# pennucci/PulsePortraiture

Hardware: AMD Instinct MI355X
Metric: subint_fits_per_sec (higher is better)
Workload: dtype f64

## Files before the change

pulseportraiture_amd/csrc/pp_common.h:

```cpp
#pragma once
#include <hip/hip_runtime.h>
#include <stdint.h>
#include <type_traits>

namespace pp {

#define PP_DCONST 4149.377593360996
#define PP_TWO_PI 6.283185307179586476925286766559
#define PP_LN10 2.302585092994045684017991454684

typedef double2 cplx;

__device__ __forceinline__ cplx cmul(cplx a, cplx b) {
    return make_double2(fma(a.x, b.x, -a.y * b.y), fma(a.x, b.y, a.y * b.x));
}
__device__ __forceinline__ cplx cmulc(cplx a, cplx b) {
    return make_double2(fma(a.x, b.x, a.y * b.y), fma(a.y, b.x, -a.x * b.y));
}
__device__ __forceinline__ cplx cadd(cplx a, cplx b) { return make_double2(a.x + b.x, a.y + b.y); }
__device__ __forceinline__ cplx csub(cplx a, cplx b) { return make_double2(a.x - b.x, a.y - b.y); }
__device__ __forceinline__ cplx cmul_mi(cplx a) { return make_double2(a.y, -a.x); }
__device__ __forceinline__ double cnorm(cplx a) { return fma(a.x, a.x, a.y * a.y); }

template <typename T>
__device__ __forceinline__ const T* as_global(const T* p) {
    typedef const T __attribute__((address_space(1)))* gp_t;
    return (const T*)(gp_t)(uintptr_t)p;
}

template <typename T>
__device__ __forceinline__ T load_uniform(const T* p) {
    typedef const T __attribute__((address_space(4)))* cp_t;
    return *(cp_t)(uintptr_t)p;
}

__device__ __forceinline__ double rn_pin(double r) { asm volatile("" : "+v"(r)); return r; }
__device__ __forceinline__ double mul_rn(double a, double b) { return rn_pin(a * b); }
__device__ __forceinline__ double add_rn(double a, double b) { return rn_pin(a + b); }
__device__ __forceinline__ double sub_rn(double a, double b) { return rn_pin(a - b); }

__device__ __forceinline__ double recip_ge1(double x) {
    double y = __builtin_amdgcn_rcp(x);
    y = fma(fma(-x, y, 1.0), y, y);
    y = fma(fma(-x, y, 1.0), y, y);
    return (x < 1e300) ? y : 0.0;
}

template <bool SC>
__device__ __forceinline__ double kconst(double v) {
    if (SC) asm volatile("" : "+s"(v));
    return v;
}
template <bool SC = false>
__device__ __forceinline__ void sincos_turns(double t, double* sn, double* cs) {
    const double q = rint(4.0 * t);
    const double y = fma(-0.25, q, t);
    const double u = y * y;
    double ps = kconst<SC>(0x1.aaec32af93359p-4);
    ps = fma(ps, u, kconst<SC>(-0x1.6fadb9f155744p-1));
    ps = fma(ps, u, kconst<SC>(0x1.e8f434d018d63p+1));
    ps = fma(ps, u, kconst<SC>(-0x1.e3074fde8871fp+3));
    ps = fma(ps, u, kconst<SC>(0x1.50783487ee782p+5));
    ps = fma(ps, u, kconst<SC>(-0x1.32d2cce62bd86p+6));
    ps = fma(ps, u, kconst<SC>(0x1.466bc6775aae2p+6));
    ps = fma(ps, u, kconst<SC>(-0x1.4abbce625be53p+5));
    ps = fma(ps, u, kconst<SC>(0x1.921fb54442d18p+2));
    const double s0 = ps * y;
    double pc = kconst<SC>(0x1.20c62c2f2d7f5p-2);
    pc = fma(pc, u, kconst<SC>(-0x1.b6e24f44b128fp+0));
    pc = fma(pc, u, kconst<SC>(0x1.f9d38a3763cc3p+2));
    pc = fma(pc, u, kconst<SC>(-0x1.a6d1f2a204a8cp+4));
    pc = fma(pc, u, kconst<SC>(0x1.e1f506891babbp+5));
    pc = fma(pc, u, kconst<SC>(-0x1.55d3c7e3cbffap+6));
    pc = fma(pc, u, kconst<SC>(0x1.03c1f081b5ac4p+6));
    pc = fma(pc, u, kconst<SC>(-0x1.3bd3cc9be45dep+4));
    const double c0 = fma(pc, u, 1.0);
    const int qi = (int)q;
    const bool odd = qi & 1;
    const double so = odd ? c0 : s0, co = odd ? s0 : c0;
    *sn = (qi & 2) ? -so : so;
    *cs = ((qi + 1) & 2) ? -co : co;
}

template <bool SC = false>
__device__ __forceinline__ cplx unit_phasor(double k, double phi) {
    double pfrac = phi - rint(phi);
    double prod = k * pfrac;
    double err = fma(k, pfrac, -prod);
    double r = (prod - rint(prod)) + err;
    double s, c;
    sincos_turns<SC>(r, &s, &c);
    return make_double2(c, s);
}

template <int W>
__device__ __forceinline__ double group_sum(double v) {
#pragma unroll
    for (int o = W / 2; o > 0; o >>= 1) v += __shfl_xor(v, o, 64);
    return v;
}
template <int W>
__device__ __forceinline__ double group_max(double v) {
#pragma unroll
    for (int o = W / 2; o > 0; o >>= 1) v = fmax(v, __shfl_xor(v, o, 64));
    return v;
}

__device__ __forceinline__ int wave_reduce16_index(int lane) { return (lane >> 2) & 15; }
template <int NS>
__device__ __forceinline__ double wave_reduce16(const double (&s)[NS], int lane) {
    double t8[8], t4[4], t2[2];
    const bool b5 = lane & 32, b4 = lane & 16, b3 = lane & 8, b2 = lane & 4;
#pragma unroll
    for (int j = 0; j < 8; ++j) {
        const double hi = (j + 8 < NS) ? s[j + 8] : 0.0;
        const double keep = b5 ? hi : s[j], send = b5 ? s[j] : hi;
        t8[j] = keep + __shfl_xor(send, 32, 64);
    }
#pragma unroll
    for (int j = 0; j < 4; ++j) {
        const double keep = b4 ? t8[j + 4] : t8[j], send = b4 ? t8[j] : t8[j + 4];
        t4[j] = keep + __shfl_xor(send, 16, 64);
    }
#pragma unroll
    for (int j = 0; j < 2; ++j) {
        const double keep = b3 ? t4[j + 2] : t4[j], send = b3 ? t4[j] : t4[j + 2];
        t2[j] = keep + __shfl_xor(send, 8, 64);
    }
    const double keep = b2 ? t2[1] : t2[0], send = b2 ? t2[0] : t2[1];
    double v = keep + __shfl_xor(send, 4, 64);
    v += __shfl_xor(v, 2, 64);
    v += __shfl_xor(v, 1, 64);
    return v;
}

template <int NS>
__device__ __forceinline__ double wave_reduce_lds(const double (&s)[NS], int lane, double* buf) {
    static_assert(NS <= 16, "one value per lane quad");
    const int wpos = (lane >> 4) * 17 + (lane & 15);
#pragma unroll
    for (int q = 0; q < NS; ++q) buf[q * 68 + wpos] = s[q];
    const int q = min(lane >> 2, NS - 1), part = lane & 3;
    const double* src = buf + q * 68 + part * 17;
    double v = 0.0;
#pragma unroll
    for (int t = 0; t < 16; ++t) v += src[t];
    v += __shfl_xor(v, 1, 64);
    v += __shfl_xor(v, 2, 64);
    return v;
}
#define PP_WRED_DOUBLES(NS) ((NS) * 68)

template <int NV>
__device__ inline void block_sum(double (&v)[NV], double* scratch) {
    const int lane = threadIdx.x & 63, wid = threadIdx.x >> 6, nw = blockDim.x >> 6;
#pragma unroll
    for (int i = 0; i < NV; ++i) v[i] = group_sum<64>(v[i]);
    __syncthreads();
    if (lane == 0) {
#pragma unroll
        for (int i = 0; i < NV; ++i) scratch[wid * NV + i] = v[i];
    }
    __syncthreads();
#pragma unroll
    for (int i = 0; i < NV; ++i) {
        double s = 0.0;
        for (int w = 0; w < nw; ++w) s += scratch[w * NV + i];
        v[i] = s;
    }
}

template <int NV, int C0>
__device__ __forceinline__ void wave_totals_to(const double (&v)[NV], int lane, double* dst) {
    constexpr int n = (NV - C0) < 16 ? (NV - C0) : 16;
    double part[n];
#pragma unroll
    for (int j = 0; j < n; ++j) part[j] = v[C0 + j];
    const double tot = wave_reduce16<n>(part, lane);
    if ((lane & 3) == 0 && (lane >> 2) < n) dst[C0 + (lane >> 2)] = tot;
    if constexpr (C0 + 16 < NV) wave_totals_to<NV, C0 + 16>(v, lane, dst);
}
#define PP_BSUM_DOUBLES(NW, NVMAX) (2 * (NW) * ((NVMAX) + 1))
template <int NV, int NVMAX>
__device__ __forceinline__ void block_sum_t(double (&v)[NV], double* scratch, int& flip, double* mx = nullptr) {
    static_assert(NV <= NVMAX, "scratch sized for NVMAX values");
    const int lane = threadIdx.x & 63, wid = threadIdx.x >> 6, nw = blockDim.x >> 6;
    double* buf = scratch + flip * nw * (NVMAX + 1);
    flip ^= 1;
    wave_totals_to<NV, 0>(v, lane, buf + wid * (NV + 1));
    if (mx) {
        const double m = group_max<64>(*mx);
        if (lane == 0) buf[wid * (NV + 1) + NV] = m;
    }
    __syncthreads();
#pragma unroll
    for (int i = 0; i < NV; ++i) {
        double s = 0.0;
        for (int w = 0; w < nw; ++w) s += buf[w * (NV + 1) + i];
        v[i] = s;
    }
    if (mx) {
        double m = buf[NV];
        for (int w = 1; w < nw; ++w) m = fmax(m, buf[w * (NV + 1) + NV]);
        *mx = m;
    }
}

struct SubState {
    double x[5];
    double xe[5];
    double f;
    double g[5];
    double H[25];
    double f0, g0[5], H0[25];
    double radius;
    double pred_red;
    int hits_boundary;
    int iter, nfev, status, done, cur;
    int npass;
    double xl[5], fl, gl[5], Hl[25];
    int fresh;
    int recentred;
    int nmodel;
    int model;
    double xprev[5];
    double geo[4];
};

#define PP_NACC 21
constexpr int PP_CHUNK_CHANNELS = 256;
#define PP_NCS 9
#define PP_TJ 10
#define PP_TSTRIDE (PP_TJ + 2)
#define PP_TAY_PAIR_STRIDE 2
__device__ __forceinline__ size_t tay_idx(size_t row, int q) { return row * PP_TSTRIDE + (size_t)q; }

}
```

pulseportraiture_amd/csrc/pp_xspec1024q.h:

```cpp
#pragma once
#include "pp_fftq.h"


namespace pp {

constexpr unsigned PP_TICKET_WINDOW_NUM = 3u, PP_TICKET_WINDOW_DEN = 4u;
__device__ __forceinline__ int ticket_moment(const long long nrows) {
    const unsigned share = (unsigned)(nrows / (long long)gridDim.x) + 1u;
    return 1 + (int)(((blockIdx.x * 2654435761u) >> 8) % (share * PP_TICKET_WINDOW_NUM / PP_TICKET_WINDOW_DEN + 1u));
}

template <int M, typename Tin>
__device__ __forceinline__ const Tin* next_row_of(const XspecArgs& a, const unsigned more_nx, const int i_nx, const int n_nx,
                                                  const size_t rc) {
    const size_t rn = more_nx ? (size_t)sub_of(a.act, i_nx) * a.nchan_full + (a.coff + n_nx * a.cstep) : rc;
    return reinterpret_cast<const Tin*>(a.data) + rn * (2 * M);
}

constexpr int FFTQ_FREE_ELEM0 = 3 * 272 + 16, FFTQ_FREE_PITCH = 17;

template <int M, bool TAIL, bool ONE = true>
__device__ __forceinline__ void store_row_results(const XspecArgs& a, const size_t rc, const int tid, double tv) {
    constexpr int H = M + 1, kc = (int)(0.75 * H);
  if constexpr (ONE) {
    const int q = wave_reduce16_index(tid);
    const double th = 0.5 * tv;
    double val = (q <= PP_TJ && ((q & 3) == 1 || (q & 3) == 2)) ? -th : th;
    double* dst = a.tay + tay_idx(rc, q < PP_TSTRIDE ? q : 0);
    if (q >= PP_TSTRIDE) { val = tv; dst = a.sdraw + rc; }
    if (TAIL) {
        const double nz = sqrt(tv / (2.0 * M) / (double)(H - kc));
        if (q > PP_TSTRIDE) { val = nz; dst = a.noise + rc; }
    }
    typedef double __attribute__((address_space(1)))* gdp_t;
    *(gdp_t)(uintptr_t)dst = val;
  } else {
    if ((tid & 3) == 0) {
        const int q = wave_reduce16_index(tid);
        if (q < PP_TSTRIDE) {
            tv *= 0.5;
            a.tay[tay_idx(rc, q)] = (q <= PP_TJ && ((q & 3) == 1 || (q & 3) == 2)) ? -tv : tv;
        }
    }
    if (tid == 4 * PP_TSTRIDE) a.sdraw[rc] = tv;
    if (TAIL && tid == 4 * (PP_TSTRIDE + 1)) a.noise[rc] = sqrt(tv / (2.0 * M) / (double)(H - kc));
  }
}

__device__ __forceinline__ void first_row_landed() { __builtin_amdgcn_s_waitcnt(0x0F70); }

constexpr int Q_PREFETCH_F64 = 1, Q_PREFETCH_F32 = 0;
template <typename Tin, bool TAIL>
__global__ __launch_bounds__(64, 2) void k_xspec_q1024(XspecArgs a) {
    constexpr int M = 1024, T = 64, R1 = 16, PER1 = 1;
    constexpr int NSL = 7;
    typedef typename RawOf<Tin>::type Raw;
    constexpr int NRED = PP_TSTRIDE + (TAIL ? 2 : 1);
    static_assert(NRED <= 16, "wave_reduce_lds takes 16 values");
    constexpr int WRED = PP_WRED_DOUBLES(NRED) / 2;
    constexpr int LDSN = WRED > FFTQ_LDS_ELEMS ? WRED : FFTQ_LDS_ELEMS;
    static_assert(2 * LDSN >= PP_TAIL_LDS_DOUBLES, "tail_work's layout of this kernel's LDS");
    constexpr bool F64 = sizeof(Tin) == 8;
    constexpr int NML = (F64 && TAIL) ? 2 : 0;
    constexpr bool TWL = F64 && !TAIL, TWR = F64 && TAIL;
    constexpr bool ROWTOP = !TAIL;
    constexpr int NTW = TWL ? 2 : 0;
    __shared__ cplx lds[LDSN + 64 * (NML + NTW)];
    static_assert(sizeof(lds) <= 19456, "eight workgroups per CU");
    static_assert(FFTQ_FREE_ELEM0 + 15 * FFTQ_FREE_PITCH < FFTQ_LDS_ELEMS && FFTQ_FREE_ELEM0 >= 64 * (TAIL ? 12 : 7) &&
                  2 * FFTQ_FREE_ELEM0 >= PP_WRED_DOUBLES(NRED), "t2's elements are outside everything a row writes");
    cplx* const ldsm = lds + LDSN + threadIdx.x;
    int tid = threadIdx.x;
    const long long nrows = (long long)a.nsub * a.nchan;
    Raw cur[PER1][R1];
    cplx t1 = a.twB[2 * tid], t2 = a.twB[32 * (tid & 15)];
    const int lam0 = fftq_lambda(tid);
    cplx wb0 = a.twB[lam0 ? lam0 : 64];
    const cplx wbT = a.twB[64];
    cplx* const ldt2 = lds + FFTQ_FREE_ELEM0;
    cplx* const ldtw = lds + LDSN + 64 * NML;
    auto put_lane_consts = [&](const cplx p1, const cplx p2, const cplx pb) {
        if (!TWL) return;
        ldt2[FFTQ_FREE_PITCH * (tid & 15)] = p2;
        ldtw[tid] = p1;
        ldtw[64 + tid] = pb;
        lds_sync<T>();
    };
    put_lane_consts(t1, t2, wb0);
    int tail_after = 0x7fffffff;
    if (a.tail) tail_after = ticket_moment(nrows);
    RowWalk<true> rw;
    rw.start(nrows, a.mwords, a.ticket, a.ticket_base);
    long long row = rw.row;
    int n = 0, i = 0;
    if (rw.more) {
        n = __builtin_amdgcn_readfirstlane((int)(row / a.nsub));
        i = __builtin_amdgcn_readfirstlane((int)(row % a.nsub));
        const size_t rc = (size_t)sub_of(a.act, i) * a.nchan_full + (a.coff + n * a.cstep);
        stage_load_global<M, T, R1>(cur, reinterpret_cast<const Tin*>(a.data) + rc * (2 * M), tid);
    }
    cplx mv2[NSL];
    const cplx* mheld = nullptr;
    const cplx* mrow = nullptr;
    int n_held = -1, ktn = 0;
    int i_nx = i, n_nx = n;
    if (ROWTOP) first_row_landed();
#pragma unroll 1
    for (int phase = 0; phase < 2; ++phase) {
    if (phase == 1) {
        if (!a.tail) break;
        tail_work(a.tail, reinterpret_cast<double*>(lds), 2 * (LDSN + 64 * NML), tid, 1);
        tail_after = 0x7fffffff;
        if (TWL) {
            const int lamr = fftq_lambda(tid);
            put_lane_consts(as_global(a.twB)[2 * tid], as_global(a.twB)[32 * (tid & 15)], as_global(a.twB)[lamr ? lamr : 64]);
        }
    }
    for (; rw.more && tail_after != 0; rw.advance(), row = rw.row, i = i_nx, n = n_nx, --tail_after) {
        rw.draw(a.ticket);
        rw.peek(nrows, a.ticket_base, a.mwords);
        asm volatile("" : "+v"(tid));
        const int lam = fftq_lambda(tid);
        const bool l0 = (lam == 0);
        const int kb = l0 ? 64 : lam;
        if (TWR) {
            t1 = as_global(a.twB)[2 * tid];
            t2 = as_global(a.twB)[32 * (tid & 15)];
            wb0 = as_global(a.twB)[kb];
        } else if (!TWL) {
            asm volatile("" : "+v"(t1.x), "+v"(t1.y), "+v"(t2.x), "+v"(t2.y), "+v"(wb0.x), "+v"(wb0.y));
        }
        const int ia = sub_of(a.act, i), ne = a.coff + n * a.cstep;
        const size_t rc = (size_t)ia * a.nchan_full + ne;
        if (channel_lookup(a, ia, n, ne, M, n_held, mrow, ktn) && mrow != mheld) {
#pragma unroll
            for (int j = 0; j < NSL; ++j) {
                const cplx mval = mrow[kb + 64 * j - 1];
                if (j < NSL - NML) mv2[j] = mval; else ldsm[64 * (j - (NSL - NML))] = mval;
            }
            mheld = mrow;
        }
        const double phin = ROWTOP ? load_uniform(a.ph0 + rc) : a.ph0[rc];
        double sd = 0.0;
        cplx v[R1];
#pragma unroll
        for (int k = 0; k < R1; ++k) v[k] = to_cplx(cur[0][k]);
        constexpr bool HALVES = F64;
        const Tin* nxrow = nullptr;
        auto load_some = [&](int k0, int k1) { load_row_pieces<Raw>(cur, nxrow, tid, k0, k1); };
        rw.next(i, n, i_nx, n_nx, nrows, a.nsub, a.ticket_base, a.ticket, a.mwords);
        nxrow = next_row_of<M, Tin>(a, rw.more_nx, i_nx, n_nx, rc);
        auto prefetch = [&]() {
            __builtin_amdgcn_sched_barrier(0);
            load_some(0, HALVES ? R1 / 2 : R1);
            __builtin_amdgcn_sched_barrier(0);
        };
        fftq1024_from<(sizeof(Tin) == 8 ? Q_PREFETCH_F64 : Q_PREFETCH_F32)>(
            v, lds, [&]() { return NTW ? ldtw[tid] : t1; }, [&]() { return TWL ? ldt2[FFTQ_FREE_PITCH * (tid & 15)] : t2; },
            tid, &sd, prefetch);
        __builtin_amdgcn_sched_barrier(0);
        {
            cplx* pub = lds + tid;
#pragma unroll
            for (int r = 0; r < NSL; ++r) pub[64 * r] = v[9 + r];
            if (TAIL) {
#pragma unroll
                for (int r = 0; r < 5; ++r) pub[64 * (NSL + r)] = v[r];
            }
            lds_sync<T>();
        }
        if (NTW) wb0 = ldtw[64 + tid];
        double tail = 0.0;
        if (TAIL) {
            const double h = 0.70710678118654752440;
            const cplx* pt = lds + fftq_lane_of((64 - lam) & 63) + (l0 ? 64 : 0);
            cplx wt = l0 ? make_double2(-h, -h) : cmul(wb0, make_double2(-h, -h));
#pragma unroll
            for (int kd = 12; kd < 16; ++kd) {
                tail += cnorm(split_pair(v[kd], pt[64 * (NSL + 15 - kd)], wt));
                wt = cmul(wt, wbT);
            }
            tail *= 0.25;
            if (tid == 0) { const double dM = v[0].x - v[0].y; tail += dM * dM; }
        }
        if (HALVES) {
            __builtin_amdgcn_sched_barrier(0);
            load_some(R1 / 2, R1);
            __builtin_amdgcn_sched_barrier(0);
        }
        const cplx* pc = lds + fftq_lane_of((64 - lam) & 63);
        const cplx el = unit_phasor<true>((double)kb, phin);
        const cplx wst = make_double2(bcast_lane0(el.x), bcast_lane0(el.y));
        cplx e = el, wb = wb0;
        const int ktu = __builtin_amdgcn_readfirstlane(ktn);
        const double kap0 = PP_TWO_PI * (double)kb;
        double tm[PP_TSTRIDE];
        cplx zc_nx = pc[64 * 6];
#pragma unroll
        for (int j = 0; j < NSL; ++j) {
            if (j > 0 && !(64 * j < ktu)) break;
            const cplx zc = zc_nx;
            if (j + 1 < NSL && 64 * (j + 1) < ktu) zc_nx = pc[64 * (5 - j)];
            if (j == 0 || 64 * j < ktu) {
                const cplx dd = split_pair(csel(l0, v[j + 1], v[j]), zc, wb);
                const cplx mj = (j < NSL - NML) ? mv2[j < NSL - NML ? j : 0] : ldsm[64 * (j - (NSL - NML))];
                const cplx x = cmulc(dd, mj);
                const cplx z = cmul(x, e);
                const double kap = j == 0 ? kap0 : kap0 + kconst<true>(PP_TWO_PI * (double)(64 * j));
                taylor_terms(j == 0, tm, x, z, kap);
            }
            if (j + 1 < NSL && 64 * (j + 1) < ktu) {
                wb = cmul(wb, wbT);
                e = cmul(e, wst);
            }
        }
        double tr[NRED];
#pragma unroll
        for (int j = 0; j < PP_TSTRIDE; ++j) tr[j] = tm[j];
        tr[PP_TSTRIDE] = sd;
        if (TAIL) tr[NRED - 1] = tail;
        lds_sync<T>();
        double tv = wave_reduce_lds(tr, tid, reinterpret_cast<double*>(lds));
        store_row_results<M, TAIL, ROWTOP>(a, rc, tid, tv);
        lds_sync<T>();
    }
    }
    if (a.tail) tail_work(a.tail, reinterpret_cast<double*>(lds), 2 * (LDSN + 64 * NML), tid, 1 << 30);
}


constexpr int PP_QF512_WPS = 3;
template <int M, typename Tin, bool TAIL>
__global__ __launch_bounds__(64, (M == 1024 ? 2 : PP_QF512_WPS)) void k_xspec_qf(XspecArgs a) {
    typedef FftQ<M> Q;
    constexpr int T = 64, R1 = Q::R, PER1 = 1;
    constexpr int NSL = R1;
    constexpr int JT = (3 * NSL) / 4;
    static_assert((int)(0.75 * (M + 1)) == 64 * JT, "the noise tail starts on a slot boundary");
    typedef typename RawOf<Tin>::type Raw;
    constexpr int NRED = PP_TSTRIDE + (TAIL ? 2 : 1);
    constexpr int WRED = PP_WRED_DOUBLES(NRED) / 2;
    constexpr int LDSN0 = Q::LDS_ELEMS > 64 * NSL ? Q::LDS_ELEMS : 64 * NSL;
    constexpr int LDSN = WRED > LDSN0 ? WRED : LDSN0;
    static_assert(M != 1024 || 2 * LDSN >= PP_TAIL_LDS_DOUBLES, "tail_work's layout of this kernel's LDS");
    __shared__ cplx lds[LDSN];
    int tid = threadIdx.x;
    constexpr bool QTOP = M == 1024 && !TAIL;
    const long long nrows = (long long)a.nsub * a.nchan;
    Raw cur[PER1][R1];
    const cplx wbT = a.twB[64];
    int tail_after = 0x7fffffff;
    if (M == 1024 && a.tail) tail_after = ticket_moment(nrows);
    RowWalk<true> rw;
    rw.start(nrows, a.mwords, a.ticket, a.ticket_base);
    long long row = rw.row;
    int n = 0, i = 0;
    if (rw.more) {
        n = __builtin_amdgcn_readfirstlane((int)(row / a.nsub));
        i = __builtin_amdgcn_readfirstlane((int)(row % a.nsub));
        const size_t rc = (size_t)sub_of(a.act, i) * a.nchan_full + (a.coff + n * a.cstep);
        stage_load_global<M, T, R1>(cur, reinterpret_cast<const Tin*>(a.data) + rc * (2 * M), tid);
    }
    int i_nx = i, n_nx = n;
    const cplx* mrow = nullptr;
    int n_held = -1, ktn = 0;
    constexpr bool MHOLD = M == 512;
    cplx mv[NSL];
    const cplx* mheld = nullptr;
    if (QTOP) first_row_landed();
#pragma unroll 1
    for (int phase = 0; phase < 2; ++phase) {
    if (phase == 1) {
        if (!(M == 1024 && a.tail)) break;
        tail_work(a.tail, reinterpret_cast<double*>(lds), 2 * LDSN, tid, 1);
        tail_after = 0x7fffffff;
    }
    for (; rw.more && tail_after != 0; rw.advance(), row = rw.row, i = i_nx, n = n_nx, --tail_after) {
        rw.draw(a.ticket);
        rw.peek(nrows, a.ticket_base, a.mwords);
        asm volatile("" : "+v"(tid));
        const int lam = Q::lambda(tid);
        const bool l0 = (lam == 0);
        const int kb = l0 ? 64 : lam;
        const cplx wb0 = as_global(a.twB)[kb];
        const int ia = sub_of(a.act, i), ne = a.coff + n * a.cstep;
        const size_t rc = (size_t)ia * a.nchan_full + ne;
        const bool looked = channel_lookup(a, ia, n, ne, M, n_held, mrow, ktn);
        if (MHOLD && looked && mrow != mheld) {
#pragma unroll
            for (int j = 0; j < NSL; ++j) mv[j] = mrow[kb + 64 * j - 1];
            mheld = mrow;
        }
        const double phin = QTOP ? load_uniform(a.ph0 + rc) : a.ph0[rc];
        double sd = 0.0;
        cplx v[R1];
#pragma unroll
        for (int k = 0; k < R1; ++k) v[k] = to_cplx(cur[0][k]);
        auto template_loads = [&]() {
            if (MHOLD) return;
            __builtin_amdgcn_sched_barrier(0);
#pragma unroll
            for (int j = 0; j < NSL; ++j) mv[j] = mrow[kb + 64 * j - 1];
            __builtin_amdgcn_sched_barrier(0);
        };
        Q::template run<3>(v, lds, as_global(a.twB), tid, &sd, template_loads);
        __builtin_amdgcn_sched_barrier(0);
        {
            cplx* pub = lds + tid;
#pragma unroll
            for (int s = 0; s < NSL; ++s) pub[64 * s] = v[s];
            lds_sync<T>();
        }
        const Tin* nxrow;
        auto load_some = [&](int k0, int k1) { load_row_pieces<Raw>(cur, nxrow, tid, k0, k1); };
        {
            __builtin_amdgcn_sched_barrier(0);
            rw.next(i, n, i_nx, n_nx, nrows, a.nsub, a.ticket_base, a.ticket, a.mwords);
            nxrow = next_row_of<M, Tin>(a, rw.more_nx, i_nx, n_nx, rc);
            load_some(0, R1 / 2);
            __builtin_amdgcn_sched_barrier(0);
        }
        const cplx* pc = lds + Q::lane_of((64 - lam) & 63);
        const cplx el = unit_phasor<true>((double)kb, phin);
        const cplx wst = make_double2(bcast_lane0(el.x), bcast_lane0(el.y));
        cplx e = el, wb = wb0;
        const int ktu = __builtin_amdgcn_readfirstlane(ktn);
        const double kap0 = PP_TWO_PI * (double)kb;
        double tm[PP_TSTRIDE];
        double tail = 0.0;
        cplx zc_nx = pc[64 * (NSL - 1)];
#pragma unroll
        for (int j = 0; j < NSL; ++j) {
            if (!TAIL && j > NSL / 2 && !(64 * j < ktu)) break;
            const cplx zc = zc_nx;
            if (j + 1 < NSL && (TAIL || 64 * (j + 1) < ktu)) zc_nx = pc[64 * (NSL - 2 - j)];
            if (j == NSL / 2) {
                __builtin_amdgcn_sched_barrier(0);
                load_some(R1 / 2, R1);
                __builtin_amdgcn_sched_barrier(0);
            }
            const bool keep = (j == 0 || 64 * j < ktu);
            if (keep || (TAIL && j >= JT - 1)) {
                const cplx dd = split_pair(csel(l0, v[(j + 1) & (NSL - 1)], v[j]), zc, wb);
                if (TAIL && j >= JT - 1) {
                    const double pw = cnorm(dd);
                    tail += (j >= JT || l0) ? pw : 0.0;
                }
              if (keep) {
                const cplx x = cmulc(dd, mv[j]);
                const cplx z = cmul(x, e);
                const double kap = j == 0 ? kap0 : kap0 + kconst<true>(PP_TWO_PI * (double)(64 * j));
                taylor_terms(j == 0, tm, x, z, kap);
              }
            }
            if (TAIL || (j + 1 < NSL && 64 * (j + 1) < ktu)) {
                wb = cmul(wb, wbT);
                e = cmul(e, wst);
            }
        }
        double tr[NRED];
#pragma unroll
        for (int j = 0; j < PP_TSTRIDE; ++j) tr[j] = tm[j];
        tr[PP_TSTRIDE] = sd;
        if (TAIL) tr[NRED - 1] = 0.25 * tail;
        lds_sync<T>();
        double tv = wave_reduce_lds(tr, tid, reinterpret_cast<double*>(lds));
        store_row_results<M, TAIL, QTOP>(a, rc, tid, tv);
        lds_sync<T>();
    }
    }
    if (M == 1024 && a.tail) tail_work(a.tail, reinterpret_cast<double*>(lds), 2 * LDSN, tid, 1 << 30);
}

}
```

Before: 74320.

## Pack per-lane constants into one word, table-drive row stores, use DPP quad reductions

```diff
diff --git a/pulseportraiture_amd/csrc/pp_common.h b/pulseportraiture_amd/csrc/pp_common.h
--- a/pulseportraiture_amd/csrc/pp_common.h
+++ b/pulseportraiture_amd/csrc/pp_common.h
@@ -134,7 +134,19 @@
     return v;
 }
 
-template <int NS>
+__device__ __forceinline__ double quad_xor1(double v) {
+    int lo = __double2loint(v), hi = __double2hiint(v);
+    lo = __builtin_amdgcn_update_dpp(lo, lo, 0xB1, 0xF, 0xF, false);
+    hi = __builtin_amdgcn_update_dpp(hi, hi, 0xB1, 0xF, 0xF, false);
+    return __hiloint2double(hi, lo);
+}
+__device__ __forceinline__ double quad_xor2(double v) {
+    int lo = __double2loint(v), hi = __double2hiint(v);
+    lo = __builtin_amdgcn_update_dpp(lo, lo, 0x4E, 0xF, 0xF, false);
+    hi = __builtin_amdgcn_update_dpp(hi, hi, 0x4E, 0xF, 0xF, false);
+    return __hiloint2double(hi, lo);
+}
+template <int NS, bool QUAD = false>
 __device__ __forceinline__ double wave_reduce_lds(const double (&s)[NS], int lane, double* buf) {
     static_assert(NS <= 16, "one value per lane quad");
     const int wpos = (lane >> 4) * 17 + (lane & 15);
@@ -145,8 +157,13 @@
     double v = 0.0;
 #pragma unroll
     for (int t = 0; t < 16; ++t) v += src[t];
-    v += __shfl_xor(v, 1, 64);
-    v += __shfl_xor(v, 2, 64);
+    if (QUAD) {
+        v += quad_xor1(v);
+        v += quad_xor2(v);
+    } else {
+        v += __shfl_xor(v, 1, 64);
+        v += __shfl_xor(v, 2, 64);
+    }
     return v;
 }
 #define PP_WRED_DOUBLES(NS) ((NS) * 68)
diff --git a/pulseportraiture_amd/csrc/pp_xspec1024q.h b/pulseportraiture_amd/csrc/pp_xspec1024q.h
--- a/pulseportraiture_amd/csrc/pp_xspec1024q.h
+++ b/pulseportraiture_amd/csrc/pp_xspec1024q.h
@@ -45,6 +45,58 @@
     if (tid == 4 * PP_TSTRIDE) a.sdraw[rc] = tv;
     if (TAIL && tid == 4 * (PP_TSTRIDE + 1)) a.noise[rc] = sqrt(tv / (2.0 * M) / (double)(H - kc));
   }
+}
+
+struct alignas(16) RowStoreEntry { float mult; unsigned stride; double* base; };
+static_assert(sizeof(RowStoreEntry) == sizeof(cplx), "one image element per entry");
+constexpr int FFTQ_STORE_ELEM0 = 2 * 272 + 16;
+__device__ __forceinline__ void put_row_store_entry(const XspecArgs& a, cplx* lds, const int tid) {
+    const int q = wave_reduce16_index(tid);
+    RowStoreEntry e;
+    if (q < PP_TSTRIDE) {
+        e.mult = (q <= PP_TJ && ((q & 3) == 1 || (q & 3) == 2)) ? -0.5f : 0.5f;
+        e.stride = (unsigned)(PP_TSTRIDE * sizeof(double));
+        e.base = a.tay + q;
+    } else {
+        e.mult = 1.0f;
+        e.stride = (unsigned)sizeof(double);
+        e.base = a.sdraw;
+    }
+    reinterpret_cast<RowStoreEntry*>(lds + FFTQ_STORE_ELEM0)[FFTQ_FREE_PITCH * q] = e;
+}
+__device__ __forceinline__ void store_row_results_lds(const cplx* lds, const size_t rc, const int tid, const double tv) {
+    const RowStoreEntry e = reinterpret_cast<const RowStoreEntry*>(lds + FFTQ_STORE_ELEM0)[FFTQ_FREE_PITCH * wave_reduce16_index(tid)];
+    char* dst = reinterpret_cast<char*>(e.base) + (unsigned long long)(unsigned)rc * e.stride;
+    typedef double __attribute__((address_space(1)))* gdp_t;
+    *(gdp_t)(uintptr_t)dst = tv * (double)e.mult;
+}
+
+__device__ __forceinline__ int fftq_lane_word(const int tid) {
+    const int lam = fftq_lambda(tid);
+    return (tid << 4) | (fftq_lane_of((64 - lam) & 63) << 14) | ((lam ? lam : 64) << 20);
+}
+__device__ __forceinline__ int lane_word_tid(const int lw) { return (lw >> 4) & 63; }
+__device__ __forceinline__ int lane_word_kb(const int lw) { return (lw >> 20) & 127; }
+__device__ __forceinline__ const cplx* lane_word_partner(const cplx* lds, const int lw) {
+    return reinterpret_cast<const cplx*>(reinterpret_cast<const char*>(lds) + ((lw >> 10) & 0x3ff));
+}
+
+template <typename Raw, int R>
+__device__ __forceinline__ void load_row_pieces_sbase(Raw (&cur)[1][R], const void* nxrow, unsigned boff, const int k0, const int k1) {
+    constexpr size_t REACH = 4096, PIECE = 64 * sizeof(Raw);
+    asm volatile("" : "+v"(boff));
+    constexpr int PER = (int)(REACH / PIECE);
+    static_assert(PER >= 1 && R % PER == 0, "whole groups of pieces: a piece within a base's reach, no piece left over");
+#pragma unroll
+    for (int g = 0; g < R / PER; ++g) {
+        if (PER * (g + 1) <= k0 || PER * g >= k1) continue;
+        const char* gg = reinterpret_cast<const char*>(nxrow) + (size_t)g * REACH;
+        asm("" : "+s"(gg));
+        gg = as_global(gg);
+#pragma unroll
+        for (int k = PER * g; k < PER * (g + 1); ++k)
+            if (k >= k0 && k < k1) cur[0][k] = load_row_once<Raw>(gg + (size_t)(k - PER * g) * PIECE + boff);
+    }
 }
 
 __device__ __forceinline__ void first_row_landed() { __builtin_amdgcn_s_waitcnt(0x0F70); }
@@ -69,24 +121,30 @@
     static_assert(sizeof(lds) <= 19456, "eight workgroups per CU");
     static_assert(FFTQ_FREE_ELEM0 + 15 * FFTQ_FREE_PITCH < FFTQ_LDS_ELEMS && FFTQ_FREE_ELEM0 >= 64 * (TAIL ? 12 : 7) &&
                   2 * FFTQ_FREE_ELEM0 >= PP_WRED_DOUBLES(NRED), "t2's elements are outside everything a row writes");
-    cplx* const ldsm = lds + LDSN + threadIdx.x;
-    int tid = threadIdx.x;
+    constexpr bool RSL = !TAIL;
+    static_assert(!RSL || (FFTQ_STORE_ELEM0 >= 64 * NSL && 2 * FFTQ_STORE_ELEM0 >= PP_WRED_DOUBLES(NRED) &&
+                           FFTQ_STORE_ELEM0 + 15 * FFTQ_FREE_PITCH < FFTQ_FREE_ELEM0),
+                  "the store entries are outside everything a row writes");
+    int lw = fftq_lane_word(threadIdx.x);
     const long long nrows = (long long)a.nsub * a.nchan;
     Raw cur[PER1][R1];
-    cplx t1 = a.twB[2 * tid], t2 = a.twB[32 * (tid & 15)];
-    const int lam0 = fftq_lambda(tid);
-    cplx wb0 = a.twB[lam0 ? lam0 : 64];
+    cplx t1 = a.twB[2 * threadIdx.x], t2 = a.twB[32 * (threadIdx.x & 15)];
+    cplx wb0 = a.twB[lane_word_kb(lw)];
     const cplx wbT = a.twB[64];
     cplx* const ldt2 = lds + FFTQ_FREE_ELEM0;
     cplx* const ldtw = lds + LDSN + 64 * NML;
+    auto put_store_entries = [&]() {
+        if (RSL) put_row_store_entry(a, lds, lane_word_tid(lw));
+    };
     auto put_lane_consts = [&](const cplx p1, const cplx p2, const cplx pb) {
-        if (!TWL) return;
+        const int tid = lane_word_tid(lw);
         ldt2[FFTQ_FREE_PITCH * (tid & 15)] = p2;
         ldtw[tid] = p1;
         ldtw[64 + tid] = pb;
-        lds_sync<T>();
     };
-    put_lane_consts(t1, t2, wb0);
+    put_store_entries();
+    if (TWL) put_lane_consts(t1, t2, wb0);
+    lds_sync<T>();
     int tail_after = 0x7fffffff;
     if (a.tail) tail_after = ticket_moment(nrows);
     RowWalk<true> rw;
@@ -97,7 +155,7 @@
         n = __builtin_amdgcn_readfirstlane((int)(row / a.nsub));
         i = __builtin_amdgcn_readfirstlane((int)(row % a.nsub));
         const size_t rc = (size_t)sub_of(a.act, i) * a.nchan_full + (a.coff + n * a.cstep);
-        stage_load_global<M, T, R1>(cur, reinterpret_cast<const Tin*>(a.data) + rc * (2 * M), tid);
+        stage_load_global<M, T, R1>(cur, reinterpret_cast<const Tin*>(a.data) + rc * (2 * M), (int)threadIdx.x);
     }
     cplx mv2[NSL];
     const cplx* mheld = nullptr;
@@ -109,20 +167,23 @@
     for (int phase = 0; phase < 2; ++phase) {
     if (phase == 1) {
         if (!a.tail) break;
-        tail_work(a.tail, reinterpret_cast<double*>(lds), 2 * (LDSN + 64 * NML), tid, 1);
+        tail_work(a.tail, reinterpret_cast<double*>(lds), 2 * (LDSN + 64 * NML), lane_word_tid(lw), 1);
         tail_after = 0x7fffffff;
+        put_store_entries();
         if (TWL) {
-            const int lamr = fftq_lambda(tid);
-            put_lane_consts(as_global(a.twB)[2 * tid], as_global(a.twB)[32 * (tid & 15)], as_global(a.twB)[lamr ? lamr : 64]);
-        }
+            const int tidr = lane_word_tid(lw);
+            put_lane_consts(as_global(a.twB)[2 * tidr], as_global(a.twB)[32 * (tidr & 15)], as_global(a.twB)[lane_word_kb(lw)]);
+        }
+        if (RSL || TWL) lds_sync<T>();
     }
     for (; rw.more && tail_after != 0; rw.advance(), row = rw.row, i = i_nx, n = n_nx, --tail_after) {
         rw.draw(a.ticket);
         rw.peek(nrows, a.ticket_base, a.mwords);
-        asm volatile("" : "+v"(tid));
-        const int lam = fftq_lambda(tid);
-        const bool l0 = (lam == 0);
-        const int kb = l0 ? 64 : lam;
+        asm volatile("" : "+v"(lw));
+        const int tid = lane_word_tid(lw);
+        const int kb = lane_word_kb(lw);
+        const bool l0 = (kb == 64);
+        cplx* const ldsm = lds + LDSN + tid;
         if (TWR) {
             t1 = as_global(a.twB)[2 * tid];
             t2 = as_global(a.twB)[32 * (tid & 15)];
@@ -147,7 +208,7 @@
         for (int k = 0; k < R1; ++k) v[k] = to_cplx(cur[0][k]);
         constexpr bool HALVES = F64;
         const Tin* nxrow = nullptr;
-        auto load_some = [&](int k0, int k1) { load_row_pieces<Raw>(cur, nxrow, tid, k0, k1); };
+        auto load_some = [&](int k0, int k1) { load_row_pieces_sbase<Raw>(cur, nxrow, (unsigned)tid * (unsigned)sizeof(Raw), k0, k1); };
         rw.next(i, n, i_nx, n_nx, nrows, a.nsub, a.ticket_base, a.ticket, a.mwords);
         nxrow = next_row_of<M, Tin>(a, rw.more_nx, i_nx, n_nx, rc);
         auto prefetch = [&]() {
@@ -173,7 +234,7 @@
         double tail = 0.0;
         if (TAIL) {
             const double h = 0.70710678118654752440;
-            const cplx* pt = lds + fftq_lane_of((64 - lam) & 63) + (l0 ? 64 : 0);
+            const cplx* pt = lane_word_partner(lds, lw) + (l0 ? 64 : 0);
             cplx wt = l0 ? make_double2(-h, -h) : cmul(wb0, make_double2(-h, -h));
 #pragma unroll
             for (int kd = 12; kd < 16; ++kd) {
@@ -188,7 +249,7 @@
             load_some(R1 / 2, R1);
             __builtin_amdgcn_sched_barrier(0);
         }
-        const cplx* pc = lds + fftq_lane_of((64 - lam) & 63);
+        const cplx* pc = lane_word_partner(lds, lw);
         const cplx el = unit_phasor<true>((double)kb, phin);
         const cplx wst = make_double2(bcast_lane0(el.x), bcast_lane0(el.y));
         cplx e = el, wb = wb0;
@@ -220,12 +281,13 @@
         tr[PP_TSTRIDE] = sd;
         if (TAIL) tr[NRED - 1] = tail;
         lds_sync<T>();
-        double tv = wave_reduce_lds(tr, tid, reinterpret_cast<double*>(lds));
-        store_row_results<M, TAIL, ROWTOP>(a, rc, tid, tv);
+        double tv = wave_reduce_lds<NRED, true>(tr, tid, reinterpret_cast<double*>(lds));
+        if (RSL) store_row_results_lds(lds, rc, tid, tv);
+        else store_row_results<M, TAIL, ROWTOP>(a, rc, tid, tv);
         lds_sync<T>();
     }
     }
-    if (a.tail) tail_work(a.tail, reinterpret_cast<double*>(lds), 2 * (LDSN + 64 * NML), tid, 1 << 30);
+    if (a.tail) tail_work(a.tail, reinterpret_cast<double*>(lds), 2 * (LDSN + 64 * NML), lane_word_tid(lw), 1 << 30);
 }
 
 
```

Result: no change. 74940 (median of 6 runs) (+0.8%).
